# latentnetworks/vimure

Measured on NVIDIA B200. Metric: cavi_ties_per_s, higher is better.
Workload: dtype f32 storage / f64 accumulate

## Files before the change

### vimure_b200/csrc/vm_kernels.cu

```cuda
#include <stdio.h>
#include <stdlib.h>

#include "vm_common.cuh"

#ifndef VM_TU_ID
#error "compile through vimure_b200/build.py (VM_TU_ID / VM_DISPATCH_CASES must be defined)"
#endif
#define VM_PASTE2(a, b) a##b
#define VM_PASTE(a, b) VM_PASTE2(a, b)
namespace VM_PASTE(vmtu, VM_TU_ID) {

static bool vm_debug_sync() {
  static int v = -1;
  if (v < 0) {
    const char* e = getenv("VM_DEBUG_SYNC");
    v = (e && e[0] == '1') ? 1 : 0;
  }
  return v == 1;
}
#define VM_CHECK_LAUNCH()                                                                          \
  do {                                                                                             \
    cudaError_t e__ = cudaGetLastError();                                                          \
    if (e__ == cudaSuccess && vm_debug_sync()) e__ = cudaDeviceSynchronize();                      \
    if (e__ != cudaSuccess) {                                                                      \
// ... 759 lines not shown
            for (int k = 0; k < K; ++k) val += erho[k] * (Gth * s_Gl[k] + z2);
          }
          t2_acc += x * log(val + eps);
        }
#pragma unroll
        for (int k = 0; k < K; ++k) cat_acc += rho[k] * (logpr[k] - log(rho[k] + eps));
        cat_acc -= (double)vm_formula_cat<K>(f, epsr, dead, cat_lp0, cat_lpk, epsf);
      }
    }
    if (RMODE == VM_R_EGO) vm_fix_accumulate<K>(fix_l, ego_diag, valid, lrow, i, j, ti, tj, o_dk, o_resid);
  }
  const int64_t nup = c.L * c.n_ublk * 8, b = ((int64_t)l * c.n_ublk + blk) * 8 + (threadIdx.x >> 5);
  const int lane = threadIdx.x & 31;
  double v;
  v = warp_sum(nu_acc);
  if (lane == 0) part[UP_NU * nup + b] = v;
  if (elbo) {
    v = warp_sum(cat_acc);
    if (lane == 0) part[UP_CAT * nup + b] = v;
    v = warp_sum(t2_acc);
    if (lane == 0) part[UP_T2 * nup + b] = v;
  }
#pragma unroll
  for (int k = 0; k < K; ++k) {
    v = warp_sum(p0[k]);
    if (lane == 0) part[(UP_P0(K) + k) * nup + b] = v;
  }
  if (RMODE == VM_R_ALL) {
#pragma unroll
    for (int k = 0; k < K; ++k) {
      v = warp_sum(dsum[k]);
      if (lane == 0) part[(UP_DELTA + k) * nup + b] = v;
    }
  }
  } while (LIST == 2 && (blk += (int)gridDim.x) < (int)c.n_ublk);
}


template <int K>
__device__ __forceinline__ bool vm_fast_tile(const vm_ctx& c, int l, int ct) {
  return (((c.N * K) & 3) == 0) && ((int64_t)(ct + 1) * DenseCfg<K>::TW <= c.N) && c.r_mode != VM_R_CSR &&
         !vm_may_dead<K>(c, l);
}

template <int K>
__device__ __forceinline__ int vm_tie_of(int lane, int t) {
  if (K == 2) return (t < 2) ? (2 * lane + t) : (64 + 2 * lane + (t - 2));
  if (K == 4) return 32 * t + lane;
  return 4 * lane + t;
}
template <int K>
__device__ __forceinline__ void vm_load_q4(const float* qrow_chunk, int lane, float* out) {
  if (K == 2) {
    const float2 a = *reinterpret_cast<const float2*>(qrow_chunk + 2 * lane);
    const float2 b = *reinterpret_cast<const float2*>(qrow_chunk + 64 + 2 * lane);
    out[0] = a.x; out[1] = a.y; out[2] = b.x; out[3] = b.y;
  } else if (K == 4) {
#pragma unroll
    for (int t = 0; t < 4; ++t) out[t] = qrow_chunk[32 * t + lane];
  } else {
    const float4 v = *reinterpret_cast<const float4*>(qrow_chunk + 4 * lane);
    out[0] = v.x; out[1] = v.y; out[2] = v.z; out[3] = v.w;
  }
}
template <int K>
__device__ __forceinline__ void vm_store_chunk(float* dst, int lane, const float* o, float* stage) {
  float4* d4 = reinterpret_cast<float4*>(dst);
  if (K == 2) {
    d4[lane] = make_float4(o[0], o[1], o[2], o[3]);
    d4[32 + lane] = make_float4(o[4], o[5], o[6], o[7]);
  } else if (K == 4) {
#pragma unroll
    for (int t = 0; t < 4; ++t) d4[32 * t + lane] = make_float4(o[4 * t], o[4 * t + 1], o[4 * t + 2], o[4 * t + 3]);
  } else if (K > 8) {
#pragma unroll
    for (int v = 0; v < K; ++v) d4[K * lane + v] = make_float4(o[4 * v], o[4 * v + 1], o[4 * v + 2], o[4 * v + 3]);
  } else {
    float4* s4 = reinterpret_cast<float4*>(stage);
#pragma unroll
    for (int v = 0; v < K; ++v) s4[K * lane + v] = make_float4(o[4 * v], o[4 * v + 1], o[4 * v + 2], o[4 * v + 3]);
    __syncwarp();
#pragma unroll
    for (int v = 0; v < K; ++v) d4[32 * v + lane] = s4[32 * v + lane];
    __syncwarp();
  }
}
template <int K>
struct StageCfg {
  static constexpr int FLOATS = (K == 2 || K == 4 || K > 8) ? 4 : 128 * K;
};

template <int K, bool ELBO, bool MD>
__device__ __forceinline__ void dense_quad(const float (*a)[K], const bool* valid, float* o, float* rowacc,
                                           float (*colacc)[4], float* coldead_chunk, int lane, double& cat, float lp0,
                                           float lpk, float epsf) {
#pragma unroll
  for (int t = 0; t < 4; ++t) {
    float epsr;
    bool dead;
    vm_formula_rho<K>(a[t], MD, &o[t * K], epsr, dead);
#pragma unroll
    for (int k = 1; k < K; ++k) {
      colacc[k - 1][t] += o[t * K + k];
      rowacc[k] += o[t * K + k];
    }
    if (MD && dead && valid[t]) {
      rowacc[0] += 1.f;
      atomicAdd(&coldead_chunk[vm_tie_of<K>(lane, t)], 1.f);
    }
    if (ELBO && valid[t]) cat += (double)vm_formula_cat<K>(&o[t * K], epsr, dead, lp0, lpk, epsf);
  }
}

template <int K, bool ELBO, bool STORE, bool CSR>
__global__ void __launch_bounds__(VM_DENSE_THREADS) k_dense(const __grid_constant__ vm_ctx c, double* catpart, int skip_fast, int rt0, int rtn) {
  constexpr int NCH = DenseCfg<K>::NCH, TW = DenseCfg<K>::TW, NW = VM_DENSE_THREADS / 32;
  __shared__ __align__(16) float qs[K][TW];
  __shared__ __align__(16) float colbuf[K][TW];
  __shared__ __align__(16) float stage[NW][StageCfg<K>::FLOATS];
  __shared__ double sm_red[8];
  const int N = (int)c.N, nloc = (int)c.nloc, nct = (int)c.nct, nrt = (int)c.nrt;
  const int ct = blockIdx.x;
  const int l = blockIdx.y / rtn, rt = rt0 + (blockIdx.y - l * rtn);
  const int tid = threadIdx.x, lane = tid & 31, warp = tid >> 5;
  if (skip_fast && vm_fast_tile<K>(c, l, ct)) return;
  const int jt = ct * TW;
  const int i_lo = rt * (int)c.tile_h, i_hi = min(i_lo + (int)c.tile_h, nloc);
  const bool may_dead = vm_may_dead<K>(c, l);
  const bool vec_ok = (((int64_t)N * K) & 3) == 0;
  const double* lc = c.layer_consts + (int64_t)l * VM_LC_STRIDE(K);
  const float lp0 = (float)lc[VM_LC_LP0(K)], lpk = (float)lc[VM_LC_LPK(K)], epsf = (float)c.eps;
  float cc[K], dd[K];
#pragma unroll
  for (int k = 0; k < K; ++k) {
    cc[k] = (float)lc[VM_LC_C(k)];
    dd[k] = (float)lc[VM_LC_D(K, k)];
  }
  for (int idx = tid; idx < TW; idx += VM_DENSE_THREADS) {
    const int j = jt + idx;
#pragma unroll
    for (int k = 0; k < K; ++k) {
      qs[k][idx] = (!CSR && j < N) ? __ldg(&c.tab_q[((int64_t)l * N + j) * K + k]) : -INFINITY;
      colbuf[k][idx] = 0.f;
    }
  }
  __syncthreads();

  float colacc[NCH][K - 1][4];
#pragma unroll
  for (int ch = 0; ch < NCH; ++ch)
#pragma unroll
    for (int k = 0; k < K - 1; ++k)
#pragma unroll
      for (int t = 0; t < 4; ++t) colacc[ch][k][t] = 0.f;
  double cat = 0.0;

  for (int i = i_lo + warp; i < i_hi; i += NW) {
    const int64_t lrow = (int64_t)l * nloc + i;
    int ua = 0, ub = 0;
    if (STORE) {
      ua = __ldg(&c.utile_ptr[lrow * nct + ct]);
      ub = __ldg(&c.utile_ptr[lrow * nct + ct + 1]);
    }
    float p[K];
#pragma unroll
    for (int k = 0; k < K; ++k) p[k] = CSR ? 0.f : __ldg(&c.tab_p[lrow * K + k]);
    float rowacc[K];
#pragma unroll
    for (int k = 0; k < K; ++k) rowacc[k] = 0.f;
    float* rowdst = c.rho + lrow * N * K;
#pragma unroll
    for (int ch = 0; ch < NCH; ++ch) {
      const int jc = jt + ch * 128;
      if (jc >= N) continue;
      bool valid[4];
      int jj[4];
      bool all_valid = true;
#pragma unroll
      for (int t = 0; t < 4; ++t) {
        jj[t] = jc + vm_tie_of<K>(lane, t);
        valid[t] = jj[t] < N;
        all_valid = all_valid && valid[t];
      }
      float a[4][K];
      if (CSR) {
#pragma unroll
        for (int t = 0; t < 4; ++t) {
          const float sv = valid[t] ? vm_csr_S32(c, l, lrow * N + jj[t]) : 0.f;
#pragma unroll
          for (int k = 0; k < K; ++k) a[t][k] = valid[t] ? __fmaf_rn(-sv, dd[k], cc[k]) : -INFINITY;
        }
      } else {
#pragma unroll
        for (int k = 0; k < K; ++k) {
          if (k == 0 && !may_dead) {
            a[0][0] = a[1][0] = a[2][0] = a[3][0] = 0.f;
            continue;
          }
          float qv[4];
          vm_load_q4<K>(&qs[k][ch * 128], lane, qv);
#pragma unroll
          for (int t = 0; t < 4; ++t) a[t][k] = __fadd_rn(p[k], qv[t]);
        }
      }
      float o[4 * K];
      if (may_dead)
        dense_quad<K, ELBO, true>(a, valid, o, rowacc, colacc[ch], &colbuf[0][ch * 128], lane, cat, lp0, lpk, epsf);
      else
        dense_quad<K, ELBO, false>(a, valid, o, rowacc, colacc[ch], &colbuf[0][ch * 128], lane, cat, lp0, lpk, epsf);
      if (STORE) {
        const bool chunk_full = jc + 128 <= N;
        if (vec_ok && chunk_full) {
          vm_store_chunk<K>(rowdst + (int64_t)jc * K, lane, o, stage[warp]);
        } else {
#pragma unroll
          for (int t = 0; t < 4; ++t)
            if (valid[t]) {
#pragma unroll
              for (int k = 0; k < K; ++k) rowdst[(int64_t)jj[t] * K + k] = o[t * K + k];
            }
        }
      }
    }
    if (!CSR) {
#pragma unroll
      for (int k = 0; k < K; ++k) {
        if (k == 0 && !may_dead) continue;
        const float v = warp_sum(rowacc[k]);
        if (lane == 0) c.rowpart[(lrow * nct + ct) * K + k] = v;
      }
      if (!may_dead && lane == 0) c.rowpart[(lrow * nct + ct) * K] = 0.f;
    }
    if (STORE) {
      __syncwarp();
      for (int u = ua + lane; u < ub; u += 32) {
        const int col = c.u_col[u];
#pragma unroll
        for (int k = 0; k < K; ++k) rowdst[(int64_t)col * K + k] = c.rho_u32[(int64_t)u * K + k];
      }
    }
  }
  if (!CSR) {
    for (int w = 0; w < NW; ++w) {
      if (warp == w) {
#pragma unroll
        for (int ch = 0; ch < NCH; ++ch)
#pragma unroll
          for (int k = 1; k < K; ++k)
#pragma unroll
            for (int t = 0; t < 4; ++t) colbuf[k][ch * 128 + vm_tie_of<K>(lane, t)] += colacc[ch][k - 1][t];
      }
      __syncthreads();
    }
    for (int idx = tid; idx < TW; idx += VM_DENSE_THREADS) {
      const int j = jt + idx;
      if (j < N) {
#pragma unroll
        for (int k = 0; k < K; ++k) c.colpart[(((int64_t)l * nrt + rt) * N + j) * K + k] = colbuf[k][idx];
      }
    }
  }
  if (ELBO) {
    const double v = block_sum<VM_DENSE_THREADS>(cat, sm_red);
    if (tid == 0) catpart[((int64_t)l * nrt + rt) * nct + ct] = v;
  }
}

#define VM_FAST_MAX_TILE_H 128

__device__ __forceinline__ void vm_bulk_store(void* gdst, const void* ssrc, uint32_t bytes) {
  asm volatile("cp.async.bulk.global.shared::cta.bulk_group [%0], [%1], %2;" ::"l"(gdst),
               "r"((uint32_t)__cvta_generic_to_shared(ssrc)), "r"(bytes)
               : "memory");
  asm volatile("cp.async.bulk.commit_group;" ::: "memory");
}
template <int N>
__device__ __forceinline__ void vm_bulk_wait_read() {
  asm volatile("cp.async.bulk.wait_group.read %0;" ::"n"(N) : "memory");
}
__device__ __forceinline__ void vm_bulk_wait_all() { asm volatile("cp.async.bulk.wait_group 0;" ::: "memory"); }
__device__ __forceinline__ void vm_fence_async_smem() { asm volatile("fence.proxy.async.shared::cta;" ::: "memory"); }

__device__ __forceinline__ void vm_smem_add_split(unsigned int* w, long long v) {
  atomicAdd(&w[0], (unsigned int)((unsigned long long)v & 0x3fffffull));
  atomicAdd(&w[1], (unsigned int)(int)(v >> 22));
}
__device__ __forceinline__ unsigned long long vm_smem_split_value(const unsigned int* w) {
  return (unsigned long long)((long long)(int)w[1] * 4194304ll + (long long)w[0]);
}

#define VM_TMA_NBUF 2
template <int K, bool SC = false>
struct TmaSmem {
  static constexpr int TW = DenseCfg<K>::TW, NW = VM_DENSE_THREADS / 32, TH = VM_FAST_MAX_TILE_H;
  float rowbuf[NW][VM_TMA_NBUF][TW * K];
  float qs[K - 1][TW];
  union {
    float colbuf[K - 1][TW];
    unsigned int colfix[SC ? TW : 1][K - 1][2];
  };
  float ps[K - 1][TH];
  int tp0[TH], tp1[TH];
  float lam[SC ? 4 * K + 1 : 1];
  double sm_red[8];
};

template <int K>
__device__ __forceinline__ void vm_stage_chunk(float* sb_chunk, int lane, const float* o) {
  float4* d4 = reinterpret_cast<float4*>(sb_chunk);
  if (K == 2) {
    d4[lane] = make_float4(o[0], o[1], o[2], o[3]);
    d4[32 + lane] = make_float4(o[4], o[5], o[6], o[7]);
  } else if (K == 4) {
#pragma unroll
    for (int t = 0; t < 4; ++t) d4[32 * t + lane] = make_float4(o[4 * t], o[4 * t + 1], o[4 * t + 2], o[4 * t + 3]);
  } else {
#pragma unroll
    for (int v = 0; v < K; ++v) d4[K * lane + v] = make_float4(o[4 * v], o[4 * v + 1], o[4 * v + 2], o[4 * v + 3]);
  }
}

template <int K>
__device__ __forceinline__ void vm_shortcut_tie(const float* rec, const float* ni, const float* nj, const float* lam,
                                                const float* cf, float* rho, long long* fq, float& nu, float* p0) {
  const float X = rec[1];
  const float xt = rec[2];
  const bool single = xt != 0.f, rowrep = xt > 0.f;
  const float g = single ? (rowrep ? ni[K - 1] : nj[K - 1]) : 1.f;
  const float el = single ? (rowrep ? ni[K] : nj[K]) : 0.f;
  const float z2 = lam[3 * K] * fabsf(xt);
  float f[K], iden[K];
#pragma unroll
  for (int k = 0; k < K; ++k) {
    const float z1 = g * lam[k];
    iden[k] = vm_rcp(z1 + z2);
    f[k] = single ? z1 * iden[k] : 1.f;
  }
  const float t0 = z2 * g * iden[0];
  float a[K], amax = 0.f;
#pragma unroll
  for (int k = 1; k < K; ++k) {
    const float dat = single ? X * ((t0 * iden[k] * lam[K + k]) * el + (f[k] * lam[2 * K + k] - f[0] * lam[2 * K]))
                             : X * lam[3 * K + 1 + k];
    const float qk = nj[k - 1];
    a[k] = ni[k - 1] + qk + rec[2 + k] + dat;
    amax = fmaxf(amax, a[k]);
  }
  float es[K], s = vm_ex2(-amax);
  es[0] = s;
#pragma unroll
  for (int k = 1; k < K; ++k) {
    es[k] = vm_ex2(a[k] - amax);
    s += es[k];
  }
  const float inv = vm_rcp(s);
  rho[0] = es[0] * inv;
  float nu_t = rho[0] * iden[0];
#pragma unroll
  for (int k = 1; k < K; ++k) {
    rho[k] = es[k] * inv;
    nu_t += rho[k] * iden[k];
    fq[k] = __double2ll_rn(((double)rho[k] - (double)cf[k]) * VM_FIX_SCALE);
  }
  if (single) {
    nu += X * z2 * nu_t;
  } else {
#pragma unroll
    for (int k = 0; k < K; ++k) p0[k] += rho[k] * X;
  }
}

template <int K>
struct ScRec {
  static constexpr int RS = (K == 2) ? 4 : 8;
};

template <int K>
__device__ __forceinline__ void vm_load_rec(const float* p, float* v) {
  const float4 a = __ldg(reinterpret_cast<const float4*>(p));
  v[0] = a.x; v[1] = a.y; v[2] = a.z; v[3] = a.w;
  if (K == 3) v[4] = __ldg(p + 4);
  if (K == 4) {
    const float2 b = __ldg(reinterpret_cast<const float2*>(p + 4));
    v[4] = b.x; v[5] = b.y;
  }
}

#ifndef VM_TMA_PD
#define VM_TMA_PD 2
#endif
template <int K, bool ELBO, bool SC, int PD>
__device__ __forceinline__ void dense_tma_body(const vm_ctx& c, double* catpart, int rt0, int rtn, unsigned char* smem) {
  constexpr int NCH = DenseCfg<K>::NCH, TW = DenseCfg<K>::TW, NW = VM_DENSE_THREADS / 32;
  constexpr int NT = NodeTab<K>::STRIDE, NV = SC ? K + 2 : K;
  static_assert(!(SC && ELBO), "the shortcut ties are evaluated on iterations without ELBO only");
  TmaSmem<K, SC>& S = *reinterpret_cast<TmaSmem<K, SC>*>(smem);
  const int N = (int)c.N, nloc = (int)c.nloc, nct = (int)c.nct, nrt = (int)c.nrt;
  const int ct = blockIdx.x;
  const int l = blockIdx.y / rtn, rt = rt0 + (blockIdx.y - l * rtn);
  if (!vm_fast_tile<K>(c, l, ct)) return;
  const int tid = threadIdx.x, lane = tid & 31, warp = tid >> 5;
  const int jt = ct * TW;
  const int i_lo = rt * (int)c.tile_h;
  const int nrows = min((int)c.tile_h, nloc - i_lo);
  const double* lc = c.layer_consts + (int64_t)l * VM_LC_STRIDE(K);
  const float lp0 = (float)lc[VM_LC_LP0(K)], lpk = (float)lc[VM_LC_LPK(K)], epsf = (float)c.eps;
  const bool sc = SC && lc[VM_LC_SIMPLE(K)] != 0.0;
  float nu = 0.f, p0[K];
#pragma unroll
  for (int k = 0; k < K; ++k) p0[k] = 0.f;
  double cat = 0.0;
  const float* patch_src = c.rho_u32;
  for (int idx = tid; idx < TW; idx += VM_DENSE_THREADS) {
#pragma unroll
    for (int k = 1; k < K; ++k) {
      S.qs[k - 1][idx] = __ldg(&c.tab_q[((int64_t)l * N + jt + idx) * K + k]);
      if (SC) S.colfix[idx][k - 1][0] = S.colfix[idx][k - 1][1] = 0u;
      else S.colbuf[k - 1][idx] = 0.f;
    }
  }
  for (int r = tid; r < nrows; r += VM_DENSE_THREADS) {
    const int64_t lrow = (int64_t)l * nloc + i_lo + r;
#pragma unroll
    for (int k = 1; k < K; ++k) S.ps[k - 1][r] = __ldg(&c.tab_p[lrow * K + k]);
    S.tp0[r] = __ldg(&c.utile_ptr[lrow * nct + ct]);
    S.tp1[r] = (SC && !sc) ? S.tp0[r] : __ldg(&c.utile_ptr[lrow * nct + ct + 1]);
  }
  if (SC && tid < K) {
    const double g0 = c.G_lambda[l * K], gkk = c.G_lambda[l * K + tid];
    S.lam[tid] = (float)gkk;
    S.lam[K + tid] = (float)(gkk - g0);
    S.lam[2 * K + tid] = (float)(c.Elog_lambda[l * K + tid] * VM_LOG2E);
    S.lam[3 * K + 1 + tid] = (float)lc[VM_LC_G(K, tid)];
    if (tid == 0) S.lam[3 * K] = (float)c.nu[VM_NU_G];
  }
  __syncthreads();
  float colacc[NCH][K - 1][4];
#pragma unroll
  for (int ch = 0; ch < NCH; ++ch)
#pragma unroll
    for (int k = 0; k < K - 1; ++k)
#pragma unroll
      for (int t = 0; t < 4; ++t) colacc[ch][k][t] = 0.f;
  int pq_col[PD];
  float pq_v[PD][NV], pq_rn[PD];
  auto fetch = [&](int row, int& col, float* v, float& rn) {
    col = 0;
    rn = 0.f;
#pragma unroll
    for (int k = 0; k < NV; ++k) v[k] = 0.f;
    if (row < nrows) {
      const int ua = S.tp0[row], n = S.tp1[row] - ua;
      if (SC) {
        if (n > 0) rn = __ldg(c.nodetab + ((int64_t)l * N + (int)c.row0 + i_lo + row) * NT + (lane & (NT - 1)));
        if (lane < n) vm_load_rec<K>(c.u_rec + (int64_t)(ua + lane) * ScRec<K>::RS, v);
      } else if (lane < n) {
        col = __ldg(&c.u_col[ua + lane]);
#pragma unroll
        for (int k = 0; k < K; ++k) v[k] = __ldg(&patch_src[(int64_t)(ua + lane) * K + k]);
      }
    }
  };
#pragma unroll
  for (int d = 0; d < PD; ++d) fetch(warp + d * NW, pq_col[d], pq_v[d], pq_rn[d]);
  float prev[K];
  int64_t prev_idx = -1;
#pragma unroll
  for (int k = 1; k < K; ++k) prev[k] = 0.f;
  int buf = 0;
  for (int r = warp; r < nrows; r += NW) {
    const int64_t lrow = (int64_t)l * nloc + i_lo + r;
    int pn_col;
    float pn_v[NV], pn_rn;
    fetch(r + PD * NW, pn_col, pn_v, pn_rn);
    float p[K];
#pragma unroll
    for (int k = 1; k < K; ++k) p[k] = S.ps[k - 1][r];
    float rowacc[K];
#pragma unroll
    for (int k = 1; k < K; ++k) rowacc[k] = 0.f;
    float* sb = S.rowbuf[warp][buf];
    if (lane == 0) vm_bulk_wait_read<VM_TMA_NBUF - 1>();
    __syncwarp();
#pragma unroll
    for (int ch = 0; ch < NCH; ++ch) {
      float qv[K][4];
#pragma unroll
      for (int k = 1; k < K; ++k) vm_load_q4<K>(&S.qs[k - 1][ch * 128], lane, qv[k]);
      float o[4 * K];
#pragma unroll
      for (int t = 0; t < 4; ++t) {
        float e[K], s = 0.f;
#pragma unroll
        for (int k = 1; k < K; ++k) {
          e[k] = vm_ex2(fminf(__fadd_rn(p[k], qv[k][t]), VM_CLAMP_LOG2));
          s = (k == 1) ? e[k] : __fadd_rn(s, e[k]);
        }
        const float inv = vm_rcp(__fadd_rn(1.f, s));
        o[t * K] = inv;
#pragma unroll
        for (int k = 1; k < K; ++k) {
          const float v = __fmul_rn(e[k], inv);
          o[t * K + k] = v;
          colacc[ch][k - 1][t] += v;
          rowacc[k] += v;
        }
        if (ELBO) cat += (double)vm_formula_cat<K>(&o[t * K], s, false, lp0, lpk, epsf);
      }
      vm_stage_chunk<K>(sb + ch * 128 * K, lane, o);
      if (ch < 5) {
#pragma unroll
        for (int k = 1; k < K; ++k) prev[k] += __shfl_down_sync(0xffffffffu, prev[k], 16 >> ch);
      }
    }
#pragma unroll
    for (int st = NCH; st < 5; ++st) {
#pragma unroll
      for (int k = 1; k < K; ++k) prev[k] += __shfl_down_sync(0xffffffffu, prev[k], 16 >> st);
    }
    if (prev_idx >= 0 && lane == 0) {
      c.rowpart[prev_idx] = 0.f;
#pragma unroll
      for (int k = 1; k < K; ++k) c.rowpart[prev_idx + k] = prev[k];
    }
    prev_idx = (lrow * nct + ct) * K;
#pragma unroll
    for (int k = 1; k < K; ++k) prev[k] = rowacc[k];
    __syncwarp();
    const int ua = S.tp0[r], n = S.tp1[r] - ua;
    if constexpr (SC) {
      if (n > 0) {
        float ni[K + 2];
#pragma unroll
        for (int t = 0; t < K + 2; ++t) ni[t] = __shfl_sync(0xffffffffu, pq_rn[0], t);
        long long frow[K];
#pragma unroll
        for (int k = 1; k < K; ++k) frow[k] = 0;
        for (int e = lane; e - lane < n; e += 32) {
          float rec[K + 2];
          if (e < 32) {
#pragma unroll
            for (int t = 0; t < K + 2; ++t) rec[t] = pq_v[0][t];
          } else {
#pragma unroll
            for (int t = 0; t < K + 2; ++t) rec[t] = 0.f;
            if (e < n) vm_load_rec<K>(c.u_rec + (int64_t)(ua + e) * ScRec<K>::RS, rec);
          }
          if (rec[1] > 0.f) {
            const int cj = (int)rec[0] - jt;
            float nj[K + 2];
            vm_load_rec<K>(c.nodetab + ((int64_t)l * N + jt + cj) * NT, nj);
            float* d = sb + cj * K;
            float cf[K], rho[K];
            long long fq[K];
#pragma unroll
            for (int k = 1; k < K; ++k) cf[k] = d[k];
            vm_shortcut_tie<K>(rec, ni, nj, S.lam, cf, rho, fq, nu, p0);
            const bool act_j = nj[K + 1] != 0.f;
#pragma unroll
            for (int k = 1; k < K; ++k) {
              if (act_j && fq[k] != 0) vm_smem_add_split(S.colfix[cj][k - 1], fq[k]);
              frow[k] += fq[k];
            }
#pragma unroll
            for (int k = 0; k < K; ++k) d[k] = rho[k];
            float* ru = c.rho_u32 + (int64_t)(ua + e) * K;
            if (K == 2) {
              *reinterpret_cast<float2*>(ru) = make_float2(rho[0], rho[1]);
            } else {
#pragma unroll
              for (int k = 0; k < K; ++k) ru[k] = rho[k];
            }
          }
        }
        if (ni[K + 1] != 0.f) {
#pragma unroll
          for (int k = 1; k < K; ++k) {
            long long v = frow[k];
#pragma unroll
            for (int o = 16; o > 0; o >>= 1) v += __shfl_down_sync(0xffffffffu, v, o);
            if (lane == 0 && v != 0)
              atomicAdd(reinterpret_cast<unsigned long long*>(c.fixA) + ((int64_t)l * c.M + (int)c.row0 + i_lo + r) * K + k,
                        (unsigned long long)v);
          }
        }
      }
    } else {
      if (lane < n) {
        float* d = sb + (pq_col[0] - jt) * K;
#pragma unroll
        for (int k = 0; k < K; ++k) d[k] = pq_v[0][k];
      }
      for (int e = 32 + lane; e < n; e += 32) {
        const int col = __ldg(&c.u_col[ua + e]);
        float* d = sb + (col - jt) * K;
#pragma unroll
        for (int k = 0; k < K; ++k) d[k] = __ldg(&patch_src[(int64_t)(ua + e) * K + k]);
      }
    }
    vm_fence_async_smem();
    __syncwarp();
    if (lane == 0) vm_bulk_store(c.rho + (lrow * N + jt) * K, sb, (uint32_t)(TW * K * sizeof(float)));
    buf = (buf + 1 == VM_TMA_NBUF) ? 0 : buf + 1;
#pragma unroll
    for (int d = 0; d + 1 < PD; ++d) {
      pq_col[d] = pq_col[d + 1];
      pq_rn[d] = pq_rn[d + 1];
#pragma unroll
      for (int k = 0; k < NV; ++k) pq_v[d][k] = pq_v[d + 1][k];
    }
    pq_col[PD - 1] = pn_col;
    pq_rn[PD - 1] = pn_rn;
#pragma unroll
    for (int k = 0; k < NV; ++k) pq_v[PD - 1][k] = pn_v[k];
  }
  if (prev_idx >= 0) {
#pragma unroll
    for (int k = 1; k < K; ++k) prev[k] = warp_sum(prev[k]);
    if (lane == 0) {
      c.rowpart[prev_idx] = 0.f;
#pragma unroll
      for (int k = 1; k < K; ++k) c.rowpart[prev_idx + k] = prev[k];
    }
  }
  if constexpr (SC) {
    __syncthreads();
    unsigned long long* fix_l = reinterpret_cast<unsigned long long*>(c.fixA) + (int64_t)l * c.M * K;
    for (int t = tid; t < TW * (K - 1); t += VM_DENSE_THREADS) {
      const unsigned long long v = vm_smem_split_value(&S.colfix[0][0][0] + 2 * t);
      if (v != 0ull) atomicAdd(fix_l + (int64_t)(jt + t / (K - 1)) * K + 1 + t % (K - 1), v);
    }
    __syncthreads();
    for (int idx = tid; idx < TW; idx += VM_DENSE_THREADS) {
#pragma unroll
      for (int k = 1; k < K; ++k) S.colbuf[k - 1][idx] = 0.f;
    }
    __syncthreads();
  }
  for (int w = 0; w < NW; ++w) {
    if (warp == w) {
#pragma unroll
      for (int ch = 0; ch < NCH; ++ch)
#pragma unroll
        for (int k = 1; k < K; ++k)
#pragma unroll
          for (int t = 0; t < 4; ++t) S.colbuf[k - 1][ch * 128 + vm_tie_of<K>(lane, t)] += colacc[ch][k - 1][t];
    }
    __syncthreads();
  }
  for (int idx = tid; idx < TW; idx += VM_DENSE_THREADS) {
    float* cp = c.colpart + (((int64_t)l * nrt + rt) * N + jt + idx) * K;
    cp[0] = 0.f;
#pragma unroll
    for (int k = 1; k < K; ++k) cp[k] = S.colbuf[k - 1][idx];
  }
  if (ELBO) {
    const double v = block_sum<VM_DENSE_THREADS>(cat, S.sm_red);
    if (tid == 0) catpart[((int64_t)l * nrt + rt) * nct + ct] = v;
  }
  if (sc) {
    const double vn = block_sum<VM_DENSE_THREADS>((double)nu, S.sm_red);
    if (tid == 0 && vn != 0.0)
      atomicAdd(reinterpret_cast<unsigned long long*>(c.dev_flags) + VM_FLAG_FIXNU,
                (unsigned long long)__double2ll_rn(vn * VM_FIXP_SCALE));
#pragma unroll
    for (int k = 0; k < K; ++k) {
      const double v = block_sum<VM_DENSE_THREADS>((double)p0[k], S.sm_red);
      if (tid == 0 && v != 0.0)
        atomicAdd(reinterpret_cast<unsigned long long*>(c.fixP) + l * K + k,
                  (unsigned long long)__double2ll_rn(v * VM_FIXP_SCALE));
    }
  }
  if (lane == 0) vm_bulk_wait_all();
}

template <int K, bool ELBO, int PD = VM_TMA_PD>
__global__ void __launch_bounds__(VM_DENSE_THREADS, (K == 2 || K == 4) ? 3 : 2) k_dense_tma(const __grid_constant__ vm_ctx c, double* catpart, int rt0, int rtn) {
  extern __shared__ __align__(128) unsigned char vm_tma_smem[];
  dense_tma_body<K, ELBO, false, PD>(c, catpart, rt0, rtn, vm_tma_smem);
}
template <int K, int PD = 1>
__global__ void __launch_bounds__(VM_DENSE_THREADS, (K == 2) ? 3 : 2) k_dense_sc(const __grid_constant__ vm_ctx c, int rt0, int rtn) {
  extern __shared__ __align__(128) unsigned char vm_tma_smem[];
  dense_tma_body<K, false, true, PD>(c, nullptr, rt0, rtn, vm_tma_smem);
}

template <int K>
__global__ void __launch_bounds__(256) k_patch_rest(const __grid_constant__ vm_ctx c) {
  const int l = blockIdx.y;
  const bool sc = c.layer_consts[(int64_t)l * VM_LC_STRIDE(K) + VM_LC_SIMPLE(K)] != 0.0;
  const int64_t lnt = (int64_t)c.nloc * c.nct;
  const int64_t p0 = sc ? c.cx_ptr[l] : c.utile_ptr[l * lnt], p1 = sc ? c.cx_ptr[l + 1] : c.utile_ptr[(l + 1) * lnt];
  for (int64_t p = p0 + (int64_t)blockIdx.x * blockDim.x + threadIdx.x; p < p1; p += (int64_t)gridDim.x * blockDim.x) {
    const int64_t u = sc ? c.cx_idx[p] : p;
    const int lrow = sc ? c.cx_lrow[p] : c.u_lrow[u], col = sc ? c.cx_col[p] : c.u_col[u];
    float* dst = c.rho + ((int64_t)lrow * c.N + col) * K;
#pragma unroll
    for (int k = 0; k < K; ++k) dst[k] = c.rho_u32[u * K + k];
  }
}

#define VM_A32_CAP 128
#define VM_A32_EF(K) ((3 * (K) + 3) / 4 * 4)
template <int K>
static inline size_t vm_all32_smem_bytes(int64_t M) {
  return ((size_t)2 * ((M + 3) / 4 * 4) + (size_t)8 * VM_A32_CAP * VM_A32_EF(K)) * sizeof(float);
}
template <int K>
__global__ void __launch_bounds__(256, (K <= 2) ? 4 : 3) k_all32(const __grid_constant__ vm_ctx c, double* part) {
  constexpr int EF = VM_A32_EF(K);
  extern __shared__ __align__(16) float a32_smem[];
  const int l = blockIdx.y, blk = blockIdx.x, tid = threadIdx.x;
  const int M = (int)c.M, Mp = (M + 3) / 4 * 4;
  float* s_G = a32_smem;
  float* s_El = s_G + Mp;
  const int warp = tid >> 5, lane = tid & 31;
  float* s_ent = s_El + Mp + warp * (VM_A32_CAP * EF);
  const double* lc = c.layer_consts + (int64_t)l * VM_LC_STRIDE(K);
  if (lc[VM_LC_SIMPLE(K)] == 0.0) return;
  const int nloc = (int)c.nloc, nct = (int)c.nct;
  const int u0 = c.utile_ptr[(int64_t)l * nloc * nct], u1 = c.utile_ptr[(int64_t)(l + 1) * nloc * nct];
  const bool mut = c.mutuality != 0;
  for (int m = tid; m < M; m += 256) {
    const double2 ge = *reinterpret_cast<const double2*>(c.GE_theta + 2 * ((int64_t)l * M + m));
    s_G[m] = (float)ge.x;
    s_El[m] = (float)(ge.y * VM_LOG2E);
  }
  float Gl[K], dGl[K];
  double Ell[K], base[K];
  const double g0 = c.G_lambda[l * K], S_all = lc[VM_LC_SALL(K)];
#pragma unroll
  for (int k = 0; k < K; ++k) {
    Gl[k] = (float)c.G_lambda[l * K + k];
    dGl[k] = (float)(c.G_lambda[l * K + k] - g0);
    Ell[k] = c.Elog_lambda[l * K + k] * VM_LOG2E;
    base[k] = -S_all * lc[VM_LC_D(K, k)];
  }
  const float Gnu = (float)c.nu[VM_NU_G];
  double cfv[K];
  {
    float a[K], cf[K], epsr;
    bool dead;
#pragma unroll
    for (int k = 0; k < K; ++k) a[k] = __fadd_rn(c.tab_p[((int64_t)l * nloc) * K + k], c.tab_q[((int64_t)l * c.N) * K + k]);
    vm_formula_rho<K>(a, false, cf, epsr, dead);
    double fk = 0.0;
#pragma unroll
    for (int k = 1; k < K; ++k) fk += (double)cf[k];
#pragma unroll
    for (int k = 0; k < K; ++k) cfv[k] = (k == 0) ? 1.0 - fk : (double)cf[k];
  }
  double nu_acc = 0.0, dsum[K], p0[K];
#pragma unroll
  for (int k = 0; k < K; ++k) dsum[k] = p0[k] = 0.0;
  __syncthreads();
  constexpr int TPW = VM_SPECIAL_TIES_PER_BLOCK / 8;
  const int wbase = u0 + blk * VM_SPECIAL_TIES_PER_BLOCK + warp * TPW;
  int64_t n_p0 = 0, n_p1 = 0;
  if (wbase + lane < u1) {
    n_p0 = c.u_ptr[wbase + lane];
    n_p1 = c.u_ptr[wbase + lane + 1];
  }
#pragma unroll 1
  for (int it = 0; it < TPW / 32; ++it) {
    const int gbase = wbase + it * 32;
    const int ng = max(0, min(32, u1 - gbase));
    const int64_t p0v = n_p0, p1v = n_p1;
    if (it + 1 < TPW / 32 && gbase + 32 + lane < u1) {
      n_p0 = c.u_ptr[gbase + 32 + lane];
      n_p1 = c.u_ptr[gbase + 32 + lane + 1];
    }
    if (ng == 0) break;
    const int64_t e0 = __shfl_sync(0xffffffffu, p0v, 0);
    const int n_e = (int)(__shfl_sync(0xffffffffu, p1v, ng - 1) - e0);
    const int qlo = (lane < ng) ? (int)(p0v - e0) : 0, qhi = (lane < ng) ? (int)(p1v - e0) : 0;
    const int u = gbase + lane;
    float lo[K], x0s = 0.f;
#pragma unroll
    for (int k = 0; k < K; ++k) lo[k] = 0.f;
    if (lane < ng) {
#pragma unroll
      for (int k = 0; k < K; ++k) lo[k] = c.u_lo[(int64_t)u * K + k];
      x0s = c.u_x0sum[u];
    }
    double W[K], T[K], dz[K];
#pragma unroll
    for (int k = 0; k < K; ++k) W[k] = T[k] = dz[k] = 0.0;
    for (int sl = 0; sl < n_e; sl += VM_A32_CAP) {
      const int ns = min(VM_A32_CAP, n_e - sl);
      for (int el0 = lane; el0 < ns; el0 += 64) {
        int mm[2];
        float xx[2], xt[2];
#pragma unroll
        for (int h = 0; h < 2; ++h) {
          const int el = el0 + 32 * h;
          const bool ok = el < ns;
          const int64_t e = e0 + sl + (ok ? el : 0);
          mm[h] = ok ? c.e_m[e] : 0;
          xx[h] = ok ? c.e_x[e] : 0.f;
          xt[h] = ok ? c.e_xT[e] : 0.f;
        }
#pragma unroll
        for (int h = 0; h < 2; ++h) {
          const int el = el0 + 32 * h;
          if (el >= ns) break;
          const int m = mm[h];
          const float x = xx[h], xT = xt[h];
          float o[EF];
#pragma unroll
          for (int q = 0; q < EF; ++q) o[q] = 0.f;
          const float elt = s_El[m];
          if (mut && xT != 0.f) {
            const float g = s_G[m];
            const float z2 = Gnu * xT;
            float iden[K];
#pragma unroll
            for (int k = 0; k < K; ++k) {
              const float z1 = g * Gl[k];
              iden[k] = vm_rcp(z1 + z2);
              o[k] = x * (z1 * iden[k]);
              o[2 * K + k] = x * z2 * iden[k];
            }
            const float t0 = x * z2 * g * iden[0];
            o[K] = o[0] * elt;
#pragma unroll
            for (int k = 1; k < K; ++k) o[K + k] = (t0 * iden[k] * dGl[k]) * elt;
          } else {
#pragma unroll
            for (int k = 0; k < K; ++k) o[k] = x;
            o[K] = x * elt;
          }
          float4* dst = reinterpret_cast<float4*>(s_ent + el * EF);
#pragma unroll
          for (int q = 0; q < EF / 4; ++q) dst[q] = make_float4(o[4 * q], o[4 * q + 1], o[4 * q + 2], o[4 * q + 3]);
        }
      }
      __syncwarp();
      const int qa = max(qlo, sl), qb = min(qhi, sl + ns);
      for (int q = qa; q < qb; ++q) {
        const float* v = s_ent + (q - sl) * EF;
#pragma unroll
        for (int k = 0; k < K; ++k) {
          W[k] += (double)v[k];
          T[k] += (double)v[K + k];
          dz[k] += (double)v[2 * K + k];
        }
      }
      __syncwarp();
    }
    if (lane < ng) {
      const double w0 = Ell[0] * W[0];
      double a[K], amax = 0.0;
      a[0] = 0.0;
#pragma unroll
      for (int k = 1; k < K; ++k) {
        a[k] = (double)lo[k] + base[k] + T[k] + (Ell[k] * W[k] - w0);
        amax = fmax(amax, a[k]);
      }
      const bool dead = (double)lo[0] + base[0] + T[0] + w0 + amax < (double)VM_DEAD_LOG2;
      float es[K], ssum = 0.f;
#pragma unroll
// ... 803 lines not shown
```

Measured before the change: 377.4 billion.

## Overlap first-batch shortcut ties with dense compute and cache node activity in smem

The shortcut-tie evaluation for each row's first 32 sparse entries moves into the last dense chunk. It recomputes the closed-form baseline from q and p instead of reading the staged buffer, so its math can overlap the dense exp/rcp work. Per-column activity flags are precomputed into a shared-memory bitmask with a ballot. Node q values now come from shared memory, and the g/Elog-theta entries are loaded from global memory only when the record needs them. This removes dependent global loads from the sparse loop, at the cost of more registers and a speculative tie computation that runs even when no tie exists.

```diff
diff --git a/vimure_b200/csrc/vm_kernels.cu b/vimure_b200/csrc/vm_kernels.cu
--- a/vimure_b200/csrc/vm_kernels.cu
+++ b/vimure_b200/csrc/vm_kernels.cu
@@ -1085,6 +1085,7 @@
   float ps[K - 1][TH];
   int tp0[TH], tp1[TH];
   float lam[SC ? 4 * K + 1 : 1];
+  unsigned int act[SC ? TW / 32 : 1];
   double sm_red[8];
 };
 
@@ -1154,6 +1155,21 @@
 }
 
 template <int K>
+__device__ __forceinline__ float vm_tma_closed_form(const float* p, const float* q, float* o) {
+  float e[K], s = 0.f;
+#pragma unroll
+  for (int k = 1; k < K; ++k) {
+    e[k] = vm_ex2(fminf(__fadd_rn(p[k], q[k]), VM_CLAMP_LOG2));
+    s = (k == 1) ? e[k] : __fadd_rn(s, e[k]);
+  }
+  const float inv = vm_rcp(__fadd_rn(1.f, s));
+  o[0] = inv;
+#pragma unroll
+  for (int k = 1; k < K; ++k) o[k] = __fmul_rn(e[k], inv);
+  return s;
+}
+
+template <int K>
 struct ScRec {
   static constexpr int RS = (K == 2) ? 4 : 8;
 };
@@ -1166,6 +1182,18 @@
   if (K == 4) {
     const float2 b = __ldg(reinterpret_cast<const float2*>(p + 4));
     v[4] = b.x; v[5] = b.y;
+  }
+}
+
+template <int K>
+__device__ __forceinline__ void vm_load_gtheta(const float* p, float& g, float& el) {
+  if (K == 2) {
+    const float4 a = __ldg(reinterpret_cast<const float4*>(p));
+    g = a.y;
+    el = a.z;
+  } else {
+    g = __ldg(p + K - 1);
+    el = __ldg(p + K);
   }
 }
 
@@ -1201,6 +1229,10 @@
       if (SC) S.colfix[idx][k - 1][0] = S.colfix[idx][k - 1][1] = 0u;
       else S.colbuf[k - 1][idx] = 0.f;
     }
+    if (SC) {
+      const unsigned int a = __ballot_sync(0xffffffffu, __ldg(c.nodetab + ((int64_t)l * N + jt + idx) * NT + K + 1) != 0.f);
+      if (lane == 0) S.act[idx >> 5] = a;
+    }
   }
   for (int r = tid; r < nrows; r += VM_DENSE_THREADS) {
     const int64_t lrow = (int64_t)l * nloc + i_lo + r;
@@ -1256,6 +1288,13 @@
     int pn_col;
     float pn_v[NV], pn_rn;
     fetch(r + PD * NW, pn_col, pn_v, pn_rn);
+    float gj = 0.f, ej = 0.f;
+    if (SC && pq_v[0][1] > 0.f && pq_v[0][2] < 0.f)
+      vm_load_gtheta<K>(c.nodetab + ((int64_t)l * N + (int)pq_v[0][0]) * NT, gj, ej);
+    bool ev_on = false;
+    int ev_cj = 0;
+    float ev_rho[K];
+    long long ev_fq[K];
     float p[K];
 #pragma unroll
     for (int k = 1; k < K; ++k) p[k] = S.ps[k - 1][r];
@@ -1270,21 +1309,38 @@
       float qv[K][4];
 #pragma unroll
       for (int k = 1; k < K; ++k) vm_load_q4<K>(&S.qs[k - 1][ch * 128], lane, qv[k]);
+      if (SC && ch == NCH - 1) {
+        const float* rec = pq_v[0];
+        ev_on = rec[1] > 0.f;
+        ev_cj = ev_on ? (int)rec[0] - jt : 0;
+        float ni[K + 2], nj[K + 1], qc[K], cf[K];
+#pragma unroll
+        for (int t = 0; t < K + 2; ++t) ni[t] = __shfl_sync(0xffffffffu, pq_rn[0], t);
+#pragma unroll
+        for (int k = 1; k < K; ++k) qc[k] = nj[k - 1] = S.qs[k - 1][ev_cj];
+        nj[K - 1] = gj;
+        nj[K] = ej;
+        vm_tma_closed_form<K>(p, qc, cf);
+        float nu_c = nu, p0_c[K];
+#pragma unroll
+        for (int k = 0; k < K; ++k) p0_c[k] = p0[k];
+        vm_shortcut_tie<K>(rec, ni, nj, S.lam, cf, ev_rho, ev_fq, nu_c, p0_c);
+        if (ev_on) {
+          nu = nu_c;
+#pragma unroll
+          for (int k = 0; k < K; ++k) p0[k] = p0_c[k];
+        }
+      }
       float o[4 * K];
 #pragma unroll
       for (int t = 0; t < 4; ++t) {
-        float e[K], s = 0.f;
+        float q[K];
+#pragma unroll
+        for (int k = 1; k < K; ++k) q[k] = qv[k][t];
+        const float s = vm_tma_closed_form<K>(p, q, &o[t * K]);
 #pragma unroll
         for (int k = 1; k < K; ++k) {
-          e[k] = vm_ex2(fminf(__fadd_rn(p[k], qv[k][t]), VM_CLAMP_LOG2));
-          s = (k == 1) ? e[k] : __fadd_rn(s, e[k]);
-        }
-        const float inv = vm_rcp(__fadd_rn(1.f, s));
-        o[t * K] = inv;
-#pragma unroll
-        for (int k = 1; k < K; ++k) {
-          const float v = __fmul_rn(e[k], inv);
-          o[t * K + k] = v;
+          const float v = o[t * K + k];
           colacc[ch][k - 1][t] += v;
           rowacc[k] += v;
         }
@@ -1319,27 +1375,44 @@
         long long frow[K];
 #pragma unroll
         for (int k = 1; k < K; ++k) frow[k] = 0;
-        for (int e = lane; e - lane < n; e += 32) {
+        if (ev_on) {
+          const int cj = ev_cj;
+          const bool act_j = (S.act[cj >> 5] >> (cj & 31)) & 1u;
+#pragma unroll
+          for (int k = 1; k < K; ++k) {
+            if (act_j && ev_fq[k] != 0) vm_smem_add_split(S.colfix[cj][k - 1], ev_fq[k]);
+            frow[k] = ev_fq[k];
+          }
+          float* d = sb + cj * K;
+#pragma unroll
+          for (int k = 0; k < K; ++k) d[k] = ev_rho[k];
+          float* ru = c.rho_u32 + (int64_t)(ua + lane) * K;
+          if (K == 2) {
+            *reinterpret_cast<float2*>(ru) = make_float2(ev_rho[0], ev_rho[1]);
+          } else {
+#pragma unroll
+            for (int k = 0; k < K; ++k) ru[k] = ev_rho[k];
+          }
+        }
+        for (int e = 32 + lane; e - lane < n; e += 32) {
           float rec[K + 2];
-          if (e < 32) {
-#pragma unroll
-            for (int t = 0; t < K + 2; ++t) rec[t] = pq_v[0][t];
-          } else {
-#pragma unroll
-            for (int t = 0; t < K + 2; ++t) rec[t] = 0.f;
-            if (e < n) vm_load_rec<K>(c.u_rec + (int64_t)(ua + e) * ScRec<K>::RS, rec);
-          }
+#pragma unroll
+          for (int t = 0; t < K + 2; ++t) rec[t] = 0.f;
+          if (e < n) vm_load_rec<K>(c.u_rec + (int64_t)(ua + e) * ScRec<K>::RS, rec);
           if (rec[1] > 0.f) {
             const int cj = (int)rec[0] - jt;
-            float nj[K + 2];
-            vm_load_rec<K>(c.nodetab + ((int64_t)l * N + jt + cj) * NT, nj);
+            float nj[K + 1];
+#pragma unroll
+            for (int k = 1; k < K; ++k) nj[k - 1] = S.qs[k - 1][cj];
+            nj[K - 1] = nj[K] = 0.f;
+            if (rec[2] < 0.f) vm_load_gtheta<K>(c.nodetab + ((int64_t)l * N + jt + cj) * NT, nj[K - 1], nj[K]);
             float* d = sb + cj * K;
             float cf[K], rho[K];
             long long fq[K];
 #pragma unroll
             for (int k = 1; k < K; ++k) cf[k] = d[k];
             vm_shortcut_tie<K>(rec, ni, nj, S.lam, cf, rho, fq, nu, p0);
-            const bool act_j = nj[K + 1] != 0.f;
+            const bool act_j = (S.act[cj >> 5] >> (cj & 31)) & 1u;
 #pragma unroll
             for (int k = 1; k < K; ++k) {
               if (act_j && fq[k] != 0) vm_smem_add_split(S.colfix[cj][k - 1], fq[k]);
```

Measured after the change: 385.1 billion (median of 6 runs). 2.1% higher.
